# TechPizzaDev/VorbisPizza

Hardware: AMD Instinct MI355X
Metric: decoded PCM Msamples/s (batched stereo N=2048) (higher is better)
Workload: dtype f32; 1 GPU; north_star: batched stereo 44.1 kHz N=2048 IMDCT + window + overlap-add to PCM through the fused kernel (Mdct.Reverse + OverlapBuffers + StoreContiguous, Mdct.cs:15-19 + StreamDecoder.cs:764-791, 594-638): 65536 all-long frames x 2 ch per GPU (BASELINE configs[1]'s batch taken all the way to PCM), spectra N(0, 2^-8) device-resident, planar float32 PCM out, 8 B per sample; frames_per_gpu=65536, channels=2, block_size=2048, device_state=steady: 200 untimed steps of the workload in front of the W warm-up steps

## Files before the change

vorbispizza_amd/_build.py:

```python
import os
import subprocess
import sys

_HERE = os.path.dirname(os.path.abspath(__file__))
CSRC = os.path.join(_HERE, "csrc")
LIB_DIR = os.path.join(_HERE, "lib")
LIB_PATH = os.path.join(LIB_DIR, "libvorbispizza_synth.so")
OBJ_DIR = os.path.join(LIB_DIR, "obj")

SOURCES = {
    "imdct_fast.hip": [],
    "imdct_exact.hip": ["-ffp-contract=off"],
    "synth_kernels.hip": [],
    "synth_dual.hip": [],
    "synth_pairs.hip": [],
    "synth_big.hip": [],
    "floor0.hip": ["-ffp-contract=off"],
    "vpz_context.hip": ["-ffp-contract=off"],
    "vpz_decoder.hip": ["-ffp-contract=off"],
    "synth_plan.hip": ["-ffp-contract=off"],
    "entropy.hip": ["-ffp-contract=off"],
    "pcm_pack.hip": [],
    "pcm_resample.hip": [],
    "pcm_logmel.hip": [],
    "pcm_fbank.hip": [],
    "pcm_loudness.hip": [],
    "pcm_truepeak.hip": [],
    "pcm_featpost.hip": ["-ffp-contract=off"],
}
COMMON = ["--offload-arch=gfx950", "-O3", "-std=c++17", "-fPIC", "-Wall", "-Wno-unused-function",
          "-Wno-constant-logical-operand", "-fno-strict-aliasing"]


def _hipcc():
    for cand in (os.environ.get("HIPCC"), "/opt/rocm/bin/hipcc"):
        if cand and os.path.exists(cand):
            return cand
    return "hipcc"


def _deps(src):
    deps = [src]
    if os.path.basename(src) == "synth_pairs.hip":
        deps.append(os.path.join(CSRC, "synth_dual.hip"))
    for name in os.listdir(CSRC):
        if name.endswith(".hpp"):
            deps.append(os.path.join(CSRC, name))
    deps.append(os.path.join(_HERE, "..", "include", "vorbispizza_synth.h"))
# ... 90 lines not shown
```

vorbispizza_amd/csrc/imdct_core.hpp:

```cpp
#pragma once

#include <hip/hip_runtime.h>

namespace vpz {

constexpr float kSqrtHalf = 0.70710678118654752440f;

typedef float vpz_c2 __attribute__((ext_vector_type(2)));
__device__ __forceinline__ vpz_c2 c2(float2 a) { return vpz_c2{a.x, a.y}; }
__device__ __forceinline__ float2 f2(vpz_c2 a) { return make_float2(a.x, a.y); }
__device__ __forceinline__ vpz_c2 cadd_i(vpz_c2 a, vpz_c2 d)
{
    vpz_c2 r;
    asm("v_pk_add_f32 %0, %1, %2 op_sel:[0,1] op_sel_hi:[1,0] neg_lo:[0,1]" : "=v"(r) : "v"(a), "v"(d));
    return r;
}
__device__ __forceinline__ vpz_c2 csub_i(vpz_c2 a, vpz_c2 d)
{
    vpz_c2 r;
    asm("v_pk_add_f32 %0, %1, %2 op_sel:[0,1] op_sel_hi:[1,0] neg_hi:[0,1]" : "=v"(r) : "v"(a), "v"(d));
    return r;
}
__device__ __forceinline__ vpz_c2 cmul2(vpz_c2 a, vpz_c2 b)
{
// ... 106 lines not shown
    const int g = lane >> 3, l = lane & 7;
    float2 z[8];
    float2 tw[8];
#pragma unroll
    for (int m = 0; m < 8; ++m) tw[m] = s_tw[l + 8 * m];
#pragma unroll
    for (int m = 0; m < 8; ++m) {
        float re = lane_mirror8(xa[7 - m].y, lane);
        z[m] = cmul(make_float2(re, xa[m].x), tw[m]);
    }
    radix8_inverse(z);
#pragma unroll
    for (int p = 1; p < 8; ++p) z[p] = cmul(z[p], s_twBC[l * 8 + p]);
#pragma unroll
    for (int p = 0; p < 8; ++p) scratch[72 * g + 9 * p + l] = z[p];
#pragma unroll
    for (int r = 0; r < 8; ++r) z[r] = scratch[72 * g + 9 * l + r];
    radix8_inverse(z);
    float wim[8];
#pragma unroll
    for (int q = 0; q < 8; ++q) {
        float2 w = cmul(z[q], tw[q]);
        z[q].x = w.x;
        wim[q] = -w.y;
    }
    float *h = reinterpret_cast<float *>(scratch);
#pragma unroll
    for (int q = 0; q < 8; ++q) {
        float hi = lane_mirror8(wim[7 - q], lane);
        reinterpret_cast<float2 *>(h)[g * 64 + l + 8 * q] = make_float2(z[q].x, hi);
    }
}

__device__ __forceinline__ void imdct2048_wave_x2_regs(const float2 (&xa)[8], const float2 (&xb)[8], float2 *scratch_a, float2 *scratch_b,
                                                       const float2 (&tw)[8], const float2 (&twAB)[8], const float2 (&twBC)[8], int lane)
{
    float2 za[8], zb[8];
#pragma unroll
    for (int m = 0; m < 8; ++m) {
        const float ra = lane_mirror64(xa[7 - m].y, lane), rb = lane_mirror64(xb[7 - m].y, lane);
        za[m] = cmul(make_float2(ra, xa[m].x), tw[m]);
        zb[m] = cmul(make_float2(rb, xb[m].x), tw[m]);
    }
    {
        float2 *sa = scratch_a, *sb = scratch_b;
        radix8_inverse(za);
        radix8_inverse(zb);
#pragma unroll
        for (int p = 1; p < 8; ++p) {
            za[p] = cmul(za[p], twAB[p]);
            zb[p] = cmul(zb[p], twAB[p]);
        }
        const int l0 = lane & 7, pp = lane >> 3;
#pragma unroll
        for (int p = 0; p < 8; ++p) {
            sa[72 * p + lane] = za[p];
            sb[72 * p + lane] = zb[p];
        }
#pragma unroll
        for (int l1 = 0; l1 < 8; ++l1) {
            za[l1] = sa[72 * pp + l0 + 8 * l1];
            zb[l1] = sb[72 * pp + l0 + 8 * l1];
        }
        radix8_inverse(za);
        radix8_inverse(zb);
#pragma unroll
        for (int q = 1; q < 8; ++q) {
            za[q] = cmul(za[q], twBC[q]);
            zb[q] = cmul(zb[q], twBC[q]);
        }
#pragma unroll
        for (int q = 0; q < 8; ++q) {
            sa[66 * l0 + pp + 8 * q] = za[q];
            sb[66 * l0 + pp + 8 * q] = zb[q];
        }
#pragma unroll
        for (int r = 0; r < 8; ++r) {
            za[r] = sa[66 * r + lane];
            zb[r] = sb[66 * r + lane];
        }
        radix8_inverse(za);
        radix8_inverse(zb);
    }
    float wa[8], wb[8];
#pragma unroll
    for (int q = 0; q < 8; ++q) {
        const float2 a = cmul(za[q], tw[q]), b = cmul(zb[q], tw[q]);
        za[q].x = a.x;
        wa[q] = -a.y;
        zb[q].x = b.x;
        wb[q] = -b.y;
    }
#pragma unroll
    for (int q = 0; q < 8; ++q) {
        const float ha = lane_mirror64(wa[7 - q], lane), hb = lane_mirror64(wb[7 - q], lane);
        scratch_a[lane + 64 * q] = make_float2(za[q].x, ha);
        scratch_b[lane + 64 * q] = make_float2(zb[q].x, hb);
    }
}

__device__ __forceinline__ void imdct256_wave8_x2(const float2 (&xa)[8], const float2 (&xb)[8], float2 *scratch_a,
                                                  float2 *scratch_b, const float2 *s_tw, const float2 *s_twBC, int lane)
{
    const int g = lane >> 3, l = lane & 7;
    float2 za[8], zb[8];
    float2 tw[8];
#pragma unroll
    for (int m = 0; m < 8; ++m) tw[m] = s_tw[l + 8 * m];
#pragma unroll
    for (int m = 0; m < 8; ++m) {
        const float ra = lane_mirror8(xa[7 - m].y, lane), rb = lane_mirror8(xb[7 - m].y, lane);
        za[m] = cmul(make_float2(ra, xa[m].x), tw[m]);
        zb[m] = cmul(make_float2(rb, xb[m].x), tw[m]);
    }
    radix8_inverse(za);
    radix8_inverse(zb);
#pragma unroll
    for (int p = 1; p < 8; ++p) {
        const float2 w = s_twBC[l * 8 + p];
        za[p] = cmul(za[p], w);
        zb[p] = cmul(zb[p], w);
    }
#pragma unroll
    for (int p = 0; p < 8; ++p) {
        scratch_a[72 * g + 9 * p + l] = za[p];
        scratch_b[72 * g + 9 * p + l] = zb[p];
    }
#pragma unroll
    for (int r = 0; r < 8; ++r) {
        za[r] = scratch_a[72 * g + 9 * l + r];
// ... 176 lines not shown
```

vorbispizza_amd/csrc/synth_plan.hip:

```cpp
#include <cstdio>
#include <cstdlib>
#include <cstring>

#include "synth_plan.hpp"

namespace vpz {

constexpr int kCutSkewPermille = 25;

namespace {

constexpr int64_t kNone = INT64_MAX;


struct Prev {
    bool has_prev, prev_long;
    int prev_end, prev_stop;
};
inline Prev prev_of_state(const StreamState &S) { return Prev{S.has_prev, S.prev_long, S.prev_end, S.prev_stop}; }
inline Prev prev_of(const Decoder &D, const vpz_packet *packets, int64_t p)
{
    if (p > 0 && packets[p - 1].stream == packets[p].stream) {
        const vpz_packet &pp = packets[p - 1];
        const PacketInfo &ppi = D.packet_info[pp.flags & 7];
// ... 757 lines not shown
        }
        return n;
    };
    const bool want_inline = P.cut_R > 0 && P.cut_R + 1 <= 16;
    P.run_inline = want_inline ? arena_alloc<uint8_t>(*P.A, 32 * n_runs + 32) : nullptr;
    auto inline_range = [&](size_t lo, size_t hi) {
        for (size_t i = lo; want_inline && i < hi; ++i) {
            const RunDesc &r = runs[i];
            uint8_t *dst = P.run_inline + 32 * i;
            memset(dst, 0, 32);
            if (!(r.flags & kRunCompact)) continue;
            const int64_t q = (int64_t)r.first + (r.pre_kind == kPreRecompute ? -1 : 0);
            const int n = std::min(16, r.count + (r.pre_kind == kPreRecompute ? 1 : 0));
            for (int j = 0; j < n; ++j) {
                dst[j] = P.cflags[q + j];
                dst[16 + j] = P.cmap[q + j];
            }
        }
    };
    P.chain_threads = 1;
    if (P.pool && P.pool->parties() > 1 && n_runs >= 1024) {
        const int n_threads = P.chain_threads = P.pool->parties();
        std::vector<int64_t> part((size_t)n_threads, 0);
        P.host_failed |= !P.pool->run([&](int party) {
            const size_t lo = n_runs * (size_t)party / n_threads, hi = n_runs * (size_t)(party + 1) / n_threads;
            part[(size_t)party] = chain_range(lo, hi);
            inline_range(lo, hi);
        });
        for (int64_t v : part) P.n_chained += v;
    } else {
        P.n_chained = chain_range(0, n_runs);
        inline_range(0, n_runs);
    }
}

}

bool SynthPlan::dual_usable() const
{
    if (!D.dual_ok || (facts.any_floor0 && !D.f0_fused) || (facts.ilv_seen && facts.planar_seen)) return false;
    const bool wide = facts.ilv_seen && !D.pairs;
    const bool dev_ok = mem_space == VPZ_MEM_HOST || D.residue_format == VPZ_RESIDUE_I16 || (residue_addr & (wide ? 15 : 7)) == 0;
    if (!(dev_ok && (wide ? facts.group_align_ok : facts.align2_ok))) return false;
    if (D.pairs && !D.pairs_always && (facts.ilv_seen || out_interleaved)) return false;
    return true;
}
bool SynthPlan::group_usable() const
{
    return D.group_ok && facts.group_align_ok &&
           (mem_space == VPZ_MEM_HOST || D.residue_format == VPZ_RESIDUE_I16 || (residue_addr & 15) == 0);
}

int plan_frames(SynthPlan &P, int64_t *samples_written)
{
    int rc = run_state_machine_parallel(P, samples_written);
    if (rc < 0) return rc;
    P.was_parallel = rc == 1;
    if (rc == 0 && (rc = run_state_machine(P, samples_written)) != VPZ_OK) return rc;
    const bool wants_group = P.facts.need_coupling || (P.out_interleaved && P.D.channels > 2);
    P.use_dual = P.dual_usable();
    P.use_group = !P.use_dual && P.D.group_ok && wants_group && !P.facts.any_floor0 && P.facts.group_align_ok &&
                  (P.mem_space == VPZ_MEM_HOST || (P.residue_addr & 15) == 0);
    return VPZ_OK;
}

void plan_runs(SynthPlan &P)
// ... 4 lines not shown
    Cut c;
    cut_segments(P, c);
    P.cut_by_cost = c.batches;
    const int n_segs = (int)W.cut_segs.size();
    const size_t runs_arena_mark = P.A->used;
    for (int attempt = 0; attempt < 2; ++attempt) {
        P.A->used = runs_arena_mark;
        P.n_runs = 0;
        c.reuse = c.batches && c.parties > 1 && W.cut_hint_frames == total_frames && W.cut_hint_streams == D.n_streams &&
                  W.cut_hint_R > 0;
        if (c.batches && W.cut_code.size() < (size_t)total_frames) W.cut_code.resize((size_t)total_frames);
        if (c.batches) W.s_units.assign((size_t)n_segs, 0);
        c.total_units = (c.batches && !c.reuse) ? count_units(P, c) : 8 * total_frames;
        c.R = W.cut_hint_R;
        c.run_slots = W.cut_hint_slots;
        c.single_round = false;
        if (!c.reuse) choose_run_length(P, c);
        c.min_run_frames = std::max(1, c.R - 1 - (c.R >= 16 ? c.R * kCutSkewPermille / 1000 + 2 : 0));
        P.runs_cap = (size_t)(total_frames / c.min_run_frames) + (size_t)std::max(n_segs, D.n_streams) + 1;
        P.runs = arena_alloc<RunDesc>(*P.A, P.runs_cap);
        if (D.generic) return;
        fit_target(P, c);
        if (!c.batches && !c.skew_frames && P.pool && P.pool->parties() > 1 && total_frames / std::max(1, c.R) >= 1024)
            write_runs_by_length_wide(P, c);
        else
            write_runs_per_segment(P, c);
        if (P.host_failed) { P.n_runs = 0; return; }
        if (!(c.reuse && ((int64_t)P.n_runs > c.run_slots || (int64_t)P.n_runs * 10 < W.cut_hint_runs * 9))) break;
        W.cut_hint_frames = -1;
    }
    if (c.batches && !c.reuse) W.cut_hint_runs = (int64_t)P.n_runs;
    P.cut_R = c.R;
    chain_runs(P);
    if (getenv("VPZ_HOST_PROFILE"))
        fprintf(stderr, "[vpz host] cut: %s, by %s, R %d, target %lld eighths, %zu runs for %lld slots, %d segments on %d threads, heavy below %lld, "
                        "hint (frames %lld, runs %lld), chained %lld, runs filled by %s on %d threads, chain sweep on %d threads\n",
                c.reuse ? "hint reused" : "fitted", c.batches ? "cost" : "length", c.R,
                (long long)c.target_units, P.n_runs, (long long)c.run_slots, n_segs, c.parties, (long long)c.heavy_work,
                (long long)W.cut_hint_frames, (long long)W.cut_hint_runs, (long long)P.n_chained,
                P.fill_threads > 1 ? "the pool" : "the calling thread", P.fill_threads, P.chain_threads);
}

}
```

vorbispizza_amd/csrc/synth_plan.hpp:

```cpp
#pragma once

#include <algorithm>

#include "host_pool.hpp"
#include "vpz_decoder.hpp"

namespace vpz {

struct BatchFacts {
    bool any_floor = false, any_floor0 = false, need_coupling = false;
    bool any_short = false;
    bool ilv_seen = false, planar_seen = false;
    bool group_align_ok = true;
    bool align2_ok = true;
    int64_t res_extent = 0;
    void note(const Decoder &D, const vpz_packet &pk)
    {
        const bool bf = pk.flags & VPZ_PKT_BLOCK_FLAG;
        if (!bf) any_short = true;
        res_extent = std::max(res_extent, pk.residue_offset + (int64_t)D.channels * ((bf ? D.size1 : D.size0) / 2));
        if (!(pk.flags & VPZ_PKT_NO_FLOOR)) {
            any_floor = true;
            if (D.mappings[pk.mapping].coupling_steps > 0) need_coupling = true;
            if (D.mapping_uses_floor0[pk.mapping]) any_floor0 = true;
        }
        if (pk.flags & VPZ_PKT_INTERLEAVED) { need_coupling = true; ilv_seen = true; }
        else planar_seen = true;
        if (pk.residue_offset & 3) group_align_ok = false;
        if (pk.residue_offset & 1) align2_ok = false;
    }
    void merge(const BatchFacts &o)
    {
        any_floor |= o.any_floor; any_floor0 |= o.any_floor0; need_coupling |= o.need_coupling; any_short |= o.any_short;
        ilv_seen |= o.ilv_seen; planar_seen |= o.planar_seen; group_align_ok &= o.group_align_ok; align2_ok &= o.align2_ok;
        res_extent = std::max(res_extent, o.res_extent);
    }
};

struct SynthPlan {
    Decoder &D;
    const int64_t n_packets;
    const vpz_packet *packets;
    const bool have_posts;
    const int mem_space;
    const uintptr_t residue_addr;
    const bool out_interleaved;
    const int64_t stream_out_capacity;
    PinnedArena *A = nullptr;
    HostPool *pool = nullptr;
    int parties = 1;
    int dual_waves = 1;
    bool needs_general = false;
    int64_t (*resident_slots)(const SynthPlan &) = nullptr;
    std::vector<StreamState> st;
    std::vector<uint8_t> started_with_prev, started_prev_long;
    FrameDesc *frames = nullptr;
    size_t n_frames = 0;
    uint8_t *rec_floor = nullptr;
    BatchFacts facts;
    bool was_parallel = false;
    bool use_group = false;
    bool use_dual = false;
    bool cut_by_cost = false;
    bool compact = false;
    uint8_t *cflags = nullptr, *cmap = nullptr;
    uint8_t *run_inline = nullptr;
    RunDesc *runs = nullptr;
    size_t n_runs = 0, runs_cap = 0;
    bool host_failed = false;
    int64_t n_chained = 0;
    int cut_R = 0;
    int fill_threads = 1, chain_threads = 1;

    int64_t capacity_of(int s) const
    {
        return D.stream_caps.empty() ? stream_out_capacity : std::min(stream_out_capacity, D.stream_caps[(size_t)s]);
    }
    bool dual_usable() const;
    bool group_usable() const;
};

int plan_frames(SynthPlan &P, int64_t *samples_written);
void plan_runs(SynthPlan &P);

}
```

vorbispizza_amd/csrc/vpz_decoder.hip:

```cpp
#include <algorithm>
#include <chrono>
#include <cstdio>
#include <cstdlib>
#include <cstring>
#include <new>
#include <vector>

#include "synth_plan.hpp"
#include "../../include/vorbispizza_synth_debug.h"

namespace vpz {

static const uint32_t k_inverse_db_bits[256] = {
#include "floor1_inverse_db_bits.inc"
};

constexpr size_t kZeroCopyMax = 8u << 20;
__global__ __launch_bounds__(256) void widen_i16_kernel(const int16_t *__restrict__ in, float *__restrict__ out, long n)
{
    const long stride = (long)gridDim.x * 256 * 8;
    if ((reinterpret_cast<uintptr_t>(in) & 15) == 0) {
        for (long i = ((long)blockIdx.x * 256 + threadIdx.x) * 8; i < n; i += stride) {
            if (i + 8 <= n) {
                const uint4 v = *reinterpret_cast<const uint4 *>(in + i);
// ... 129 lines not shown
    if (cfg->floor_count < 0 || cfg->mapping_count < 0 || (cfg->floor_count && !cfg->floors && !cfg->floor_types) ||
        (cfg->mapping_count && !cfg->mappings) || cfg->mapping_count > 256 || cfg->floor_count > 64)
        return set_error(ctx, VPZ_E_INVALID_ARG, "vpz_decoder_create: bad floor / mapping tables");
    VPZ_HIP_TRY(ctx, hipSetDevice(ctx->device));

    vpz_decoder *d = new (std::nothrow) vpz_decoder();
    if (!d) return VPZ_E_NOMEM;
    Decoder &D = d->impl;
    D.ctx = ctx;
    D.channels = cfg->channels;
    D.size0 = cfg->block_size0;
    D.size1 = cfg->block_size1;
    D.clip = cfg->clip_samples ? 1 : 0;
    D.n_streams = n_streams;
    {
        const char *no_big = getenv("VPZ_NO_BIG");
        D.big = synth_big_supported(cfg->block_size0, cfg->block_size1) && !(no_big && atoi(no_big));
    }
    D.generic = !synth_supports_sizes(cfg->block_size0, cfg->block_size1) && !D.big;
    D.states.assign(n_streams, StreamState());
    D.floors.assign((size_t)cfg->floor_count, vpz_floor1_config{});
    D.floor_types.assign((size_t)cfg->floor_count, 1);
    D.floors0.assign((size_t)cfg->floor_count, vpz_floor0_config{});
    for (int i = 0; i < cfg->floor_count; ++i) {
        if (cfg->floor_types) D.floor_types[i] = cfg->floor_types[i];
        if (D.floor_types[i] == 1 && cfg->floors) D.floors[i] = cfg->floors[i];
        if (D.floor_types[i] == 0 && cfg->floors0) D.floors0[i] = cfg->floors0[i];
    }
    D.mappings.assign(cfg->mappings, cfg->mappings + cfg->mapping_count);
    static_assert(VPZ_PKT_BLOCK_FLAG == 1 && VPZ_PKT_PREV_FLAG == 2 && VPZ_PKT_NEXT_FLAG == 4, "packet_info index");
    for (int f = 0; f < 8; ++f) D.packet_info[f] = get_packet_info(D.size0, D.size1, f & 1, f & 2, f & 4);
    if (const char *e = getenv("VPZ_NO_DIRECT_I16")) D.no_direct_i16 = atoi(e) != 0;
    if (const char *e = getenv("VPZ_NO_CHAIN")) D.no_chain = atoi(e) != 0;
    if (const char *e = getenv("VPZ_DUAL_RUN")) D.dual_run = std::max(4, atoi(e));
    if (const char *e = getenv("VPZ_PLAN_SLOTS")) D.plan_slots = std::max<int64_t>(0, atoll(e));
    if (const char *e = getenv("VPZ_SYNTH_ABLATE")) D.ablate = atoi(e);
    if (const char *e = getenv("VPZ_HOST_THREADS")) D.host_threads = atoi(e);
    if (const char *e = getenv("VPZ_NO_EARLY_UPLOAD")) D.no_early_upload = atoi(e) != 0;
    if (const char *e = getenv("VPZ_PAR_MIN_PACKETS")) D.par_min_packets = atoll(e);

    int rc = VPZ_OK;
    std::vector<FloorDev> fdev(std::max<size_t>(1, D.floors.size()));
    for (size_t i = 0; i < D.floors.size() && rc == VPZ_OK; ++i) {
        if (D.floor_types[i] == 1) {
            rc = build_floor(D.floors[i], &fdev[i]);
        } else if (D.floor_types[i] == 0) {
            const vpz_floor0_config &f0 = D.floors0[i];
            if (f0.order < 1 || f0.order > 255 || f0.rate < 1 || f0.bark_map_size < 1 || f0.amp_bits < 0 || f0.amp_bits > 63)
                rc = VPZ_E_INVALID_ARG;
        } else {
            rc = VPZ_E_INVALID_ARG;
        }
    }
    std::vector<uint8_t> steps;
    for (size_t m = 0; m < D.mappings.size() && rc == VPZ_OK; ++m) {
        const vpz_mapping_config &mc = D.mappings[m];
        if (mc.coupling_steps < 0 || mc.coupling_steps > VPZ_MAX_COUPLING) { rc = VPZ_E_INVALID_ARG; break; }
        while (mc.coupling_steps && steps.size() % (2 * kStepsPadPairs)) steps.push_back(0);
        D.mapping_steps_off.push_back(mc.coupling_steps ? (int32_t)steps.size() : -1);
        for (int i = 0; i < mc.coupling_steps; ++i) {
            const int mag = mc.coupling_magnitude[i], ang = mc.coupling_angle[i];
            if (mag == ang || mag >= D.channels || ang >= D.channels) { rc = VPZ_E_INVALID_ARG; break; }
            steps.push_back((uint8_t)mag);
            steps.push_back((uint8_t)ang);
        }
        for (int ch = 0; ch < D.channels && rc == VPZ_OK; ++ch)
// ... 327 lines not shown
    GenericFrame *gf = nullptr;
    int64_t *src0 = nullptr, *dst0 = nullptr, *src1 = nullptr, *dst1 = nullptr;
    int32_t *save_list = nullptr;
    size_t n0 = 0, n1 = 0, n_save = 0;
    int64_t y_floats = 0;
    const float *d_res = nullptr, *d_amp = nullptr, *d_coeff = nullptr;
    const int16_t *d_posts = nullptr;
    const uint8_t *d_counts = nullptr;
    void *d_out = nullptr;
    bool early_residue = false, early_posts = false;
    bool spec_i16 = false;
    int64_t early_res_extent = 0;

    SynthCall(Decoder &dec, int64_t n, const vpz_packet *pk, const float *res, const int16_t *po, const uint8_t *pc,
              int mem, void *out, const int64_t *out_off, int64_t out_cap, int layout, int64_t stride)
        : D(dec), ctx(dec.ctx), n_packets(n), packets(pk), residue(res), posts(po), post_counts(pc), mem_space(mem),
          pcm_out(out), stream_out_offset(out_off), stream_out_capacity(out_cap), out_layout(layout),
          channel_stride(stride), C(dec.channels), half0(dec.size0 / 2), half1(dec.size1 / 2),
          n_rec(n * dec.channels), have_posts(po && pc && !dec.floors.empty()),
          out_interleaved(layout == VPZ_OUT_INTERLEAVED || layout == VPZ_OUT_INTERLEAVED_S16),
          out_s16(layout == VPZ_OUT_INTERLEAVED_S16 || layout == VPZ_OUT_PLANAR_S16),
          out_elem(out_s16 ? sizeof(int16_t) : sizeof(float)),
          P{dec, n, pk, have_posts, mem, reinterpret_cast<uintptr_t>(res), out_interleaved, out_cap}
    {
    }

    void *dev(const void *host_ptr) const
    {
        if (!host_ptr) return nullptr;
        char *base = zero_copy ? A->mapped : static_cast<char *>(A->dev.p);
        return base + (static_cast<const char *>(host_ptr) - A->base);
    }
    bool zero_copy = false;

    int resolved_parties = 0;
    int host_parties()
    {
        if (resolved_parties > 0) return resolved_parties;
        int parties = D.host_threads;
        if (parties <= 0) {
            cpu_set_t set;
            parties = sched_getaffinity(0, sizeof set, &set) == 0 ? CPU_COUNT(&set) : (int)std::thread::hardware_concurrency();
            if (const char *lw = getenv("LOCAL_WORLD_SIZE")) parties /= std::max(1, atoi(lw));
            parties = std::max(1, std::min(parties, 16));
        }
        return resolved_parties = parties;
    }
    HostPool *own_pool()
    {
        const int parties = host_parties();
        HostPool *pool = static_cast<HostPool *>(ctx->host_pool);
        if (n_packets >= D.par_min_packets && parties >= 2 && !(pool && pool->parties() == parties)) {
            if (pool) ctx->host_pool_free(pool);
            ctx->host_pool = pool = new HostPool(parties);
            ctx->host_pool_free = [](void *p) { delete static_cast<HostPool *>(p); };
        }
        return pool && parties >= 2 && pool->parties() == parties ? pool : nullptr;
    }

    int plan_frames(int64_t *samples_written)
    {
        P.A = A;
        P.pool = own_pool();
        P.parties = host_parties();
        P.dual_waves = synth_dual_waves();
        P.needs_general = synth_needs_general(D.size0, D.size1);
// ... 382 lines not shown
        a.f0_stride = D.f0_k;
        a.spec_i16 = spec_i16 ? 1 : 0;
        a.state_h = D.d_state_h;
        if (D.big && !P.use_dual) {
            const int64_t tf = synth_big_tail_floats(D.size1, (int64_t)P.n_runs * C);
            if (tf > 0) {
                const int grc = grow(ctx, D.b_bigtail, sizeof(float) * (size_t)tf);
                if (grc != VPZ_OK) return grc;
            }
            a.big_tail = static_cast<float *>(D.b_bigtail.p);
        }
        a.state_slot_floats = (int64_t)D.n_streams * C * half1;
        a.tw_long = D.t1->d_fast;
        a.tw_short = D.t0->d_fast;
        a.slope0 = D.t0->d_slope;
        a.slope1 = D.t1->d_slope;
        a.out = static_cast<float *>(d_out);
        a.stream_out_off = d_outoff;
        a.channel_stride = dev_channel_stride;
        a.interleaved = out_interleaved;
        a.s16 = out_s16 ? 1 : 0;
        a.clip = D.clip;
        a.clipped = D.d_clipped;
        a.no_batch = ((D.ablate & 128) || !P.cut_by_cost || P.facts.any_floor0) ? 1 : 0;
        a.ablate = D.ablate;
        a.stamps = nullptr;
#if defined(VPZ_STAMPS) || defined(VPZ_WAVE_TIMES)
        static unsigned long long *d_stamps = nullptr;
        constexpr size_t kStampWaves = 1 << 16;
        if (!d_stamps) (void)hipMalloc(&d_stamps, (16 + 16 * kStampWaves) * sizeof(unsigned long long));
        (void)hipMemsetAsync(d_stamps, 0, (16 + 16 * std::min<size_t>(kStampWaves, P.n_runs)) * sizeof(unsigned long long), ctx->stream);
        a.stamps = d_stamps;
#endif
        hipError_t e = P.use_dual ? (D.pairs ? launch_synth_pairs(a, P.facts.any_floor, P.facts.ilv_seen, ctx->stream) : launch_synth_dual(a, P.facts.any_floor, P.facts.ilv_seen, ctx->stream))
                                : D.big ? launch_synth_big(a, P.facts.any_floor, ctx->stream) : launch_synth(a, P.facts.any_floor, ctx->stream);
        if (e != hipSuccess) return set_error(ctx, VPZ_E_HIP, "synth kernel launch", e);
#if defined(VPZ_STAMPS) || defined(VPZ_WAVE_TIMES)
        {
            unsigned long long h[16];
            (void)hipMemcpyAsync(h, d_stamps, sizeof(h), hipMemcpyDeviceToHost, ctx->stream);
            (void)hipStreamSynchronize(ctx->stream);
            static const char *names_one[9] = {"desc+prefetch", "barrier0", "stage+barrier", "coupling", "pickup+curve",
                                               "floor*+imdct", "wait next", "ola+stores", "tail"};
            static const char *names_dual[9] = {"desc+prefetch", "unpack+coupling", "curves", "floor*+imdct x2", "wait next",
                                                "ola+stores", "tail", "-", "-"};
            const char **names = P.use_dual ? names_dual : names_one;
            unsigned long long tot = 0;
            for (int k = 0; k < 9; ++k) tot += h[k];
            fprintf(stderr, "[stamps] %llu waves, %.0f cycles per wave:", h[15], h[15] ? (double)tot / h[15] : 0.0);
            for (int k = 0; k < 9; ++k) fprintf(stderr, " %s %.1f%%", names[k], tot ? 100.0 * h[k] / tot : 0.0);
            if (h[14] && h[15]) {
                const double mean = (double)tot / h[15], var = (double)h[13] * 1e6 / h[15] - mean * mean;
                fprintf(stderr, " | slowest wave %.0f cycles = %.2f x mean, sigma %.2f x mean, %.1f passes per wave, %d runs", (double)h[14],
                        (double)h[14] / mean, var > 0 ? sqrt(var) / mean : 0.0, (double)h[12] / h[15], (int)P.n_runs);
            }
            fprintf(stderr, "\n");
            if (const char *dump = getenv("VPZ_STAMPS_DUMP")) {
                const size_t nw = std::min<size_t>(kStampWaves, P.n_runs);
                std::vector<unsigned long long> w(16 * nw);
                (void)hipMemcpy(w.data(), d_stamps + 16, w.size() * sizeof(unsigned long long), hipMemcpyDeviceToHost);
                if (FILE *f = fopen(dump, "w")) {
                    fprintf(f, "run,stream,frames,passes,long_frames,c0,c1,c2,c3,c4,c5,c6\n");
                    for (size_t r = 0; r < nw; ++r) {
                        fprintf(f, "%zu,%d,%d,%llu,%llu", r, P.runs[r].stream, P.runs[r].count, w[16 * r + 9], w[16 * r + 10]);
                        for (int k = 0; k < 7; ++k) fprintf(f, ",%llu", w[16 * r + k]);
                        fprintf(f, "\n");
                    }
// ... 78 lines not shown
    const auto t_arena = tick();
    if ((rc = call.plan_frames(samples_written)) != VPZ_OK) return rc;
    const SynthPlan &plan = call.P;
    if (plan.facts.res_extent > residue_floats)
        return set_error(ctx, VPZ_E_INVALID_ARG, "vpz_decoder_synth: a packet's residue lies beyond residue_floats");
    const auto t_pass1 = tick();
    if (plan.n_frames == 0) {
        D.states = plan.st;
        return VPZ_OK;
    }
    plan_runs(call.P);
    if (plan.host_failed) return set_error(ctx, VPZ_E_NOMEM, "vpz_decoder_synth: run cutting failed (allocation)");
    call.build_coupling_packets();
    if ((rc = call.build_floor0_records()) != VPZ_OK) return rc;
    if ((rc = call.build_output_offsets()) != VPZ_OK) return rc;
    call.build_generic_lists();
    const auto t_pass2 = tick();
    if ((rc = call.stage_inputs()) != VPZ_OK) return rc;
    if ((rc = call.launch()) != VPZ_OK) return rc;
    if (call.zero_copy) {
        VPZ_HIP_TRY(ctx, hipEventRecord(call.A->uploaded, ctx->stream));
        call.A->pending = true;
    }
    if ((rc = call.copy_back()) != VPZ_OK) return rc;
    early_guard.completed = mem_space == VPZ_MEM_HOST;
    if (!D.generic)
        for (int s = 0; s < D.n_streams; ++s)
            if (D.plan.s_cnt[s] > 0) call.P.st[s].state_slot ^= 1;
    D.states = plan.st;
    if (host_profile) {
        const auto t_end = tick();
        auto us = [](auto a, auto b) { return std::chrono::duration<double, std::micro>(b - a).count(); };
        const char *route = D.generic ? "generic" : plan.use_dual ? (D.pairs ? "pairs" : "stereo") : D.big ? "big" : plan.use_group ? "group" : "separate";
        fprintf(stderr, "[vpz host] packets %lld: route %s, arena wait %.1f us, pass1 %.1f us (%s), runs %.1f us, uploads+launch %.1f us\n",
                (long long)n_packets, route, us(t_begin, t_arena), us(t_arena, t_pass1), plan.was_parallel ? "parallel" : "serial",
                us(t_pass1, t_pass2), us(t_pass2, t_end));
    }
    return VPZ_OK;
}

int vpz_decoder_synth(vpz_decoder *d, int64_t n_packets, const vpz_packet *packets, const float *residue,
                      int64_t residue_floats, const int16_t *posts, const uint8_t *post_counts, int64_t n_records,
                      int mem_space, void *pcm_out, const int64_t *stream_out_offset, int64_t stream_out_capacity,
                      int out_layout, int64_t channel_stride, int64_t *samples_written)
{
    if (!d) return VPZ_E_INVALID_ARG;
    try {
        return synth_impl(d, n_packets, packets, residue, residue_floats, posts, post_counts, n_records, mem_space, pcm_out,
                          stream_out_offset, stream_out_capacity, out_layout, channel_stride, samples_written);
    } catch (const ArenaOverflow &) {
        return set_error(d->impl.ctx, VPZ_E_NOMEM, "vpz_decoder_synth: the descriptor arena is too small for this batch");
    } catch (const std::bad_alloc &) {
        return set_error(d->impl.ctx, VPZ_E_NOMEM, "vpz_decoder_synth: host allocation failed");
    } catch (...) {
        return set_error(d->impl.ctx, VPZ_E_NOMEM, "vpz_decoder_synth: host pass failed");
    }
}

int vpz_decoder_last_packet_status(vpz_decoder *d, int32_t *out, int64_t capacity, int64_t *n_not_ok)
{
    if (!d || capacity < 0 || (capacity > 0 && !out)) return VPZ_E_INVALID_ARG;
    Decoder &D = d->impl;
    const int64_t n = std::min<int64_t>(capacity, (int64_t)D.packet_samples.size());
    for (int64_t i = 0; i < n; ++i) out[i] = VPZ_OK;
    for (int64_t p : D.mismatch_packets)
        if (p < n) out[p] = VPZ_E_WINDOW_MISMATCH;
    if (n_not_ok) *n_not_ok = (int64_t)D.mismatch_packets.size();
    return VPZ_OK;
// ... 152 lines not shown
```

vorbispizza_amd/csrc/vpz_decoder.hpp:

```cpp
#pragma once

#include <vector>

#include "vpz_internal.hpp"

namespace vpz {

struct StreamState {
    bool has_prev = false;
    bool prev_long = false;
    int prev_start = 0, prev_end = 0, prev_stop = 0;
    int64_t current_position = 0;
    bool has_position = true;
    bool eos_found = false;
    bool has_clipped = false;
    int32_t clip_epoch = 1;
    int32_t state_slot = 0;
};

using DevBuf = Scratch;

struct PinnedArena {
    char *base = nullptr;
    char *mapped = nullptr;
// ... 63 lines not shown
    bool pairs_always = false;
    uint8_t *d_pair_ch = nullptr;
    uint32_t *d_pair_map_bits = nullptr;
    uint8_t *d_pair_steps = nullptr;
    int n_pair_step_pairs = 0;
    int max_steps = 0, n_step_pairs = 0;
    int host_threads = 0;
    int64_t par_min_packets = 16384;
    DevBuf b_in_res, b_in_posts, b_in_counts, b_out;
    DevBuf b_in_res16;
    int residue_format = VPZ_RESIDUE_F32;
    DevBuf b_ybuf;
    DevBuf b_bigtail;
    bool generic = false;
    bool big = false;
    std::vector<uint8_t> floor_types;
    std::vector<vpz_floor0_config> floors0;
    void *d_floors0 = nullptr;
    int32_t *d_bark_maps = nullptr;
    bool f0_fused = false;
    bool has_floor1 = false;
    int f0_k = 0;
    uint16_t *d_f0_bark = nullptr;
    float *d_f0_w = nullptr;
    DevBuf b_f0curve;
    DevBuf b_in_amp, b_in_coeff;
    const float *f0_amp = nullptr, *f0_coeff = nullptr;
    int32_t f0_stride = 0;
    PacketInfo packet_info[8];
    int dual_run = 8;
    int64_t plan_slots = 0;
    bool no_direct_i16 = false;
    bool no_chain = false;
    int ablate = 0;
    bool no_early_upload = false;
    std::vector<int32_t> packet_samples;
    std::vector<int64_t> mismatch_packets;
};

}
```

vorbispizza_amd/csrc/vpz_internal.hpp:

```cpp
#pragma once

#include <hip/hip_runtime.h>

#include <array>
#include <cstdint>
#include <map>
#include <string>
#include <utility>
#include <vector>

#include "../../include/vorbispizza_synth.h"
#include "../../include/vorbispizza_pcm_pack.h"
#include "synth_desc.hpp"

namespace vpz {

struct BlockTables {
    int n = 0;
    float2 *d_fast = nullptr;
    float *d_A = nullptr, *d_B = nullptr, *d_C = nullptr;
    uint16_t *d_bitrev = nullptr;
    int ld = 0;
    float *d_slope = nullptr;
    std::vector<float> h_slope;
// ... 91 lines not shown
                                 const int64_t *src_off = nullptr, const int64_t *dst_off = nullptr);
hipError_t launch_imdct_fast_4096(const float *spectra, float *out, int64_t count, const float2 *tw, Context *ctx,
                                  hipStream_t stream, const int64_t *src_off = nullptr, const int64_t *dst_off = nullptr);
hipError_t launch_imdct_fast_8192(const float *spectra, float *out, int64_t count, const float2 *tw, Context *ctx,
                                  hipStream_t stream, const int64_t *src_off = nullptr, const int64_t *dst_off = nullptr);
hipError_t launch_imdct_fast_mid(int n, const float *spectra, float *out, int64_t count, const float2 *tw, Context *ctx,
                                 hipStream_t stream, const int64_t *src_off = nullptr,
                                 const int64_t *dst_off = nullptr);
hipError_t launch_imdct_exact(int n, int ld, const float *spectra, float *out, int64_t count,
                              const float *A, const float *B, const float *C,
                              const uint16_t *bitrev, int num_cu, hipStream_t stream,
                              const int64_t *src_off = nullptr, const int64_t *dst_off = nullptr);

hipError_t launch_floor1_unwrap(int n_rec, const int16_t *posts, const uint8_t *post_counts, const uint8_t *rec_info,
                                const FloorDev *floors, int n_floors, int32_t *cposts, uint8_t *ccount, int16_t *dbg_y,
                                uint8_t *dbg_f, hipStream_t stream, int f0_fused = 0);
hipError_t launch_floor0_curves(int n_rec, const uint8_t *rec_info, const void *floors, const float *amp, const float *coeff,
                                int coeff_stride, int k_stride, const float *wtab, float *curve, const uint8_t *post_counts,
                                uint8_t *ccount, int32_t *cposts, hipStream_t stream);
hipError_t launch_floor0_wtab(const void *floors, int n_floors, int k_stride, float *wtab, hipStream_t stream);
hipError_t launch_floor1_render(int n_rec, const int32_t *cposts, const uint8_t *ccount, const uint8_t *rec_info,
                                int half0, int half1, uint8_t *curve_y, hipStream_t stream);
hipError_t launch_coupling(const void *pkts, int n_pkts, const uint8_t *steps, int channels,
                           const float *residue, float *temp, int max_half, hipStream_t stream);
hipError_t launch_synth(const SynthArgs &args, bool has_floor, hipStream_t stream);
bool synth_supports_sizes(int size0, int size1);
bool synth_needs_general(int size0, int size1);
int synth_resident_waves(bool has_floor, int num_cu, int channels, bool group);
bool synth_group_supported(int channels);
bool synth_dual_supported(int channels, int size0, int size1);
hipError_t launch_synth_dual(const SynthArgs &args, bool has_floor, bool interleaved_in, hipStream_t stream);
int synth_dual_resident_slots(bool has_floor, int num_cu);
int synth_dual_waves();
bool synth_pairs_supported(int channels, int size0, int size1);
hipError_t launch_synth_pairs(const SynthArgs &args, bool has_floor, bool interleaved_in, hipStream_t stream);
bool synth_big_supported(int size0, int size1);
hipError_t launch_synth_big(const SynthArgs &args, bool has_floor, hipStream_t stream);
int synth_big_resident_waves(bool has_floor, int num_cu, int size0, int size1);
int64_t synth_big_tail_floats(int size1, int64_t n_items);
hipError_t launch_generic_floor(const GenericFrame *frames, int n_frames, int channels, int half1, float *spec,
                                const uint8_t *post_counts, const uint8_t *curve_y, const float *inv_db,
                                hipStream_t stream);
hipError_t launch_generic_ola(const GenericFrame *frames, int n_frames, int channels, int size0, int size1,
                              const float *ybuf, float *state_y, const float *slope0, const float *slope1, float *out,
                              const int64_t *stream_out_off, int64_t channel_stride, int interleaved, int clip,
                              int32_t *clipped, int s16, hipStream_t stream);
hipError_t launch_generic_save_state(const GenericFrame *frames, const int32_t *save_list, int n_save, int channels,
                                     int size1, const float *ybuf, float *state_y, hipStream_t stream);
hipError_t launch_floor0_apply(const void *recs, int n_recs, const void *floors, const int32_t *bark_maps,
                               const float *amp, const float *coeff, int coeff_stride, float *spec,
                               hipStream_t stream);
size_t floor0_dev_size();
size_t floor0_rec_size();
void fill_floor0_dev(void *dst, int order, int bark_map_size, int amp_ofs, int64_t off_short, int64_t off_long);
void fill_floor0_rec(void *dst, int64_t spec_off, int rec, int floor, int half, int is_long);
size_t coupling_packet_size();
void fill_coupling_packet(void *dst, int64_t src_off, int64_t dst_off, int32_t half, int32_t steps_off,
                          int32_t steps, int32_t interleaved);

constexpr int kFastTwOffset = 0;
constexpr int kFastTwABOffset = 512;
constexpr int kFastTwBCOffset = 1024;
constexpr int kFastTableCount = 1024 + 64;
constexpr int kFast4096TwOffset = 0, kFast4096TwABOffset = 1024, kFast4096TwBCOffset = 1536, kFast4096WOffset = 1600;
constexpr int kFast4096TableCount = 2112;
constexpr int kFast8192TwOffset = 0, kFast8192TwABOffset = 2048, kFast8192TwBCOffset = 2560, kFast8192W1Offset = 2624,
// ... 9 lines not shown
```

Measured before the change: 609,000 Msamples/s.

## Add specialized steady-state stereo long-block synthesis kernel with register-resident overlap-add

Adds a dedicated kernel for the all-long, floorless, planar stereo 2048 case. It keeps previous-frame tails in registers, applies the window and overlap-add directly from the IMDCT outputs via lane mirroring, and writes PCM with nontemporal paired stores, skipping the scratch round-trip of the general dual path. Cross-wave neighbour handoff goes through shared memory with a spin-wait. The host plan detects eligibility and routes to it, and a compile-time sweep verifies the index maps. This adds a specialized code path and spin synchronization that could stall if assumptions fail.

New measurement: 696,400 Msamples/s (median of 6 runs). 1.14x the previous value.

```diff
diff --git a/vorbispizza_amd/_build.py b/vorbispizza_amd/_build.py
--- a/vorbispizza_amd/_build.py
+++ b/vorbispizza_amd/_build.py
@@ -14,6 +14,7 @@
     "synth_kernels.hip": [],
     "synth_dual.hip": [],
     "synth_pairs.hip": [],
+    "steady_stereo.hip": [],
     "synth_big.hip": [],
     "floor0.hip": ["-ffp-contract=off"],
     "vpz_context.hip": ["-ffp-contract=off"],
diff --git a/vorbispizza_amd/csrc/imdct_core.hpp b/vorbispizza_amd/csrc/imdct_core.hpp
--- a/vorbispizza_amd/csrc/imdct_core.hpp
+++ b/vorbispizza_amd/csrc/imdct_core.hpp
@@ -162,8 +162,9 @@
     }
 }
 
-__device__ __forceinline__ void imdct2048_wave_x2_regs(const float2 (&xa)[8], const float2 (&xb)[8], float2 *scratch_a, float2 *scratch_b,
-                                                       const float2 (&tw)[8], const float2 (&twAB)[8], const float2 (&twBC)[8], int lane)
+__device__ __forceinline__ void imdct2048_wave_x2_spectrum(const float2 (&xa)[8], const float2 (&xb)[8], float2 *scratch_a, float2 *scratch_b,
+                                                           const float2 (&tw)[8], const float2 (&twAB)[8], const float2 (&twBC)[8], int lane,
+                                                           float (&re_a)[8], float (&nim_a)[8], float (&re_b)[8], float (&nim_b)[8])
 {
     float2 za[8], zb[8];
 #pragma unroll
@@ -212,20 +213,26 @@
         radix8_inverse(za);
         radix8_inverse(zb);
     }
-    float wa[8], wb[8];
 #pragma unroll
     for (int q = 0; q < 8; ++q) {
         const float2 a = cmul(za[q], tw[q]), b = cmul(zb[q], tw[q]);
-        za[q].x = a.x;
-        wa[q] = -a.y;
-        zb[q].x = b.x;
-        wb[q] = -b.y;
-    }
+        re_a[q] = a.x;
+        nim_a[q] = -a.y;
+        re_b[q] = b.x;
+        nim_b[q] = -b.y;
+    }
+}
+
+__device__ __forceinline__ void imdct2048_wave_x2_regs(const float2 (&xa)[8], const float2 (&xb)[8], float2 *scratch_a, float2 *scratch_b,
+                                                       const float2 (&tw)[8], const float2 (&twAB)[8], const float2 (&twBC)[8], int lane)
+{
+    float ra[8], wa[8], rb[8], wb[8];
+    imdct2048_wave_x2_spectrum(xa, xb, scratch_a, scratch_b, tw, twAB, twBC, lane, ra, wa, rb, wb);
 #pragma unroll
     for (int q = 0; q < 8; ++q) {
         const float ha = lane_mirror64(wa[7 - q], lane), hb = lane_mirror64(wb[7 - q], lane);
-        scratch_a[lane + 64 * q] = make_float2(za[q].x, ha);
-        scratch_b[lane + 64 * q] = make_float2(zb[q].x, hb);
+        scratch_a[lane + 64 * q] = make_float2(ra[q], ha);
+        scratch_b[lane + 64 * q] = make_float2(rb[q], hb);
     }
 }
 
diff --git a/vorbispizza_amd/csrc/steady_map.hpp b/vorbispizza_amd/csrc/steady_map.hpp
--- /dev/null
+++ b/vorbispizza_amd/csrc/steady_map.hpp
@@ -0,0 +1,45 @@
+#pragma once
+
+namespace vpz {
+namespace steady {
+
+constexpr int kLanes = 64, kRegs = 8;
+constexpr int point(int lane, int q) { return lane + 64 * q; }
+constexpr int tail_index(int lane, int q) { return q < 4 ? 511 - 2 * point(lane, q) : 2 * point(lane, q) - 512; }
+constexpr int cur_index(int lane, int q) { return q < 4 ? 2 * point(lane, q) : 1023 - 2 * point(lane, q); }
+constexpr int sample_lo(int k) { return 511 - k; }
+constexpr int sample_hi(int k) { return 512 + k; }
+constexpr int kept_sample(int lane, int q) { return q < 4 ? sample_hi(cur_index(lane, q)) : sample_lo(cur_index(lane, q)); }
+constexpr int sent_sample(int lane, int q) { return q < 4 ? sample_lo(cur_index(lane, q)) : sample_hi(cur_index(lane, q)); }
+constexpr int store_index(int lane, int q) { return q < 4 ? 512 + 2 * point(lane, q) : 2 * point(lane, q) - 512; }
+
+constexpr bool sweep()
+{
+    bool tail_seen[512] = {}, sample_seen[1024] = {};
+    for (int q = 0; q < kRegs; ++q)
+        for (int l = 0; l < kLanes; ++l) {
+            const int t = tail_index(l, q), k = cur_index(l, q);
+            if (t < 0 || t >= 512 || tail_seen[t]) return false;
+            tail_seen[t] = true;
+            if (k < 0 || k >= 512) return false;
+            if (t != 511 - k) return false;
+            const int a = sample_lo(k), b = sample_hi(k);
+            if (a < 0 || a >= 512 || b < 512 || b >= 1024 || sample_seen[a] || sample_seen[b]) return false;
+            sample_seen[a] = sample_seen[b] = true;
+            const int pl = 63 - l, pq = 7 - q;
+            if (kept_sample(l, q) & 1) return false;
+            if (sent_sample(pl, pq) != kept_sample(l, q) + 1) return false;
+            if (store_index(l, q) != kept_sample(l, q)) return false;
+            const int j = point(l, q), ia = 2 * j, ib = 1023 - 2 * j;
+            if (q < 4 ? (ia != k || ib != 512 + t) : (ib != k || ia != 512 + t)) return false;
+        }
+    for (int i = 0; i < 512; ++i)
+        if (!tail_seen[i]) return false;
+    for (int i = 0; i < 1024; ++i)
+        if (!sample_seen[i]) return false;
+    return true;
+}
+static_assert(sweep(), "steady_stereo_kernel's index maps: tails a permutation of 0..511, samples of 0..1023, swap partners (63 - l, 7 - q)");
+
+}
+}
diff --git a/vorbispizza_amd/csrc/steady_stereo.hip b/vorbispizza_amd/csrc/steady_stereo.hip
--- /dev/null
+++ b/vorbispizza_amd/csrc/steady_stereo.hip
@@ -0,0 +1,223 @@
+#include "imdct_core.hpp"
+#include "steady_map.hpp"
+#include "synth_common.hpp"
+#include "synth_desc.hpp"
+#include "vpz_internal.hpp"
+
+namespace vpz {
+
+constexpr int kSteadyWaves = 4;
+constexpr int kSteadyThreads = 64 * kSteadyWaves;
+
+__global__ __launch_bounds__(kSteadyThreads, 2) void steady_stereo_kernel(SynthArgs a)
+{
+    __shared__ float2 s_scr[kSteadyWaves][2][kWaveScratchFloat2];
+    __shared__ int s_done[kSteadyWaves];
+
+    const int lane = threadIdx.x & 63;
+    const int wave = __builtin_amdgcn_readfirstlane(threadIdx.x >> 6);
+    const int run_idx = (int)blockIdx.x * kSteadyWaves + wave;
+    const bool active = run_idx < a.n_runs;
+    RunDesc run = a.runs[active ? run_idx : 0];
+    float2 rtw[8], rtwAB[8], rtwBC[8];
+    float w_lo[8], w_hi[8];
+    {
+        const VPZ_GLOBAL float2 *tw = (const VPZ_GLOBAL float2 *)a.tw_long;
+        const VPZ_GLOBAL float *sl = (const VPZ_GLOBAL float *)a.slope1;
+#pragma unroll
+        for (int m = 0; m < 8; ++m) {
+            rtw[m] = tw[kFastTwOffset + lane + 64 * m];
+            rtwAB[m] = tw[kFastTwABOffset + 64 * m + lane];
+            rtwBC[m] = tw[kFastTwBCOffset + 8 * (lane & 7) + m];
+            const int k = steady::cur_index(lane, m);
+            w_lo[m] = sl[steady::sample_lo(k)];
+            w_hi[m] = sl[steady::sample_hi(k)];
+        }
+    }
+    if (threadIdx.x < kSteadyWaves) s_done[threadIdx.x] = 0;
+    __syncthreads();
+    if (!active) return;
+
+    float2 *scrL = s_scr[wave][0], *scrR = s_scr[wave][1];
+    const int n_staged = run.count + (run.pre_kind == kPreRecompute ? 1 : 0);
+    const bool defer = run.pre_kind == kPreNeighbour && wave > 0 && run.count > 0;
+    const bool first_emits = run.pre_kind == kPreState;
+    const VPZ_GLOBAL float2 *src = (const VPZ_GLOBAL float2 *)(a.spec + run.spec_base);
+    const VPZ_GLOBAL float2 *idle = (const VPZ_GLOBAL float2 *)a.inv_db;
+    float *row_l, *row_r;
+    {
+        float *ob = a.out + (a.stream_out_off ? a.stream_out_off[run.stream] : 0) + run.out_base;
+        const uint64_t p = reinterpret_cast<uint64_t>(ob);
+        const uint32_t lo = __builtin_amdgcn_readfirstlane((uint32_t)p), hi = __builtin_amdgcn_readfirstlane((uint32_t)(p >> 32));
+        row_l = reinterpret_cast<float *>(((uint64_t)hi << 32) | lo);
+        row_r = row_l + a.channel_stride;
+    }
+    const bool clip_on = a.clip != 0;
+    float clip_peak = 0.0f;
+
+    float tL[8], tR[8];
+#pragma unroll
+    for (int q = 0; q < 8; ++q) tL[q] = tR[q] = 0.0f;
+    if (run.pre_kind == kPreState) {
+        const VPZ_GLOBAL float *st = (const VPZ_GLOBAL float *)(a.state_h + (size_t)run.state_slot * a.state_slot_floats + (size_t)run.stream * 2 * 1024);
+#pragma unroll
+        for (int q = 0; q < 8; ++q) {
+            tL[q] = st[steady::tail_index(lane, q)];
+            tR[q] = st[1024 + steady::tail_index(lane, q)];
+        }
+    }
+    float parkL[8], parkR[8];
+#pragma unroll
+    for (int q = 0; q < 8; ++q) parkL[q] = parkR[q] = 0.0f;
+
+    auto prefetch = [&](const VPZ_GLOBAL float2 *s2, bool valid, float2 (&va)[8], float2 (&vb)[8]) {
+        int l = lane;
+        asm volatile("" : "+v"(l));
+        const VPZ_GLOBAL float2 *p = valid ? s2 : idle;
+        const int base = valid ? l : 0, step = valid ? 64 : 0, rofs = valid ? 512 : 0;
+#pragma unroll
+        for (int m = 0; m < 8; ++m) {
+            va[m] = p[base + step * m];
+            vb[m] = p[base + step * m + rofs];
+        }
+    };
+    auto emit = [&](const float (&curL)[8], const float (&curR)[8], const float (&pL)[8], const float (&pR)[8], float *out_l, float *out_r) {
+        float loL[8], hiL[8], loR[8], hiR[8];
+#pragma unroll
+        for (int q = 0; q < 8; ++q) {
+            loL[q] = ola(-curL[q], w_lo[q], pL[q], w_hi[q]);
+            hiL[q] = ola(curL[q], w_hi[q], pL[q], w_lo[q]);
+            loR[q] = ola(-curR[q], w_lo[q], pR[q], w_hi[q]);
+            hiR[q] = ola(curR[q], w_hi[q], pR[q], w_lo[q]);
+        }
+        if (clip_on) {
+#pragma unroll
+            for (int q = 0; q < 8; q += 2) {
+                clip_group(loL[q], hiL[q], loL[q + 1], hiL[q + 1], clip_peak);
+                clip_group(loR[q], hiR[q], loR[q + 1], hiR[q + 1], clip_peak);
+            }
+        }
+        int lf = lane;
+        asm volatile("" : "+v"(lf));
+#pragma unroll
+        for (int q = 0; q < 8; ++q) {
+            const float gotL = lane_mirror64(q < 4 ? hiL[7 - q] : loL[7 - q], lf);
+            const float gotR = lane_mirror64(q < 4 ? hiR[7 - q] : loR[7 - q], lf);
+            const int at = q < 4 ? 512 + 2 * (lf + 64 * q) : 2 * (lf + 64 * q) - 512;
+            vpz_f2v vl = {q < 4 ? hiL[q] : loL[q], gotL}, vr = {q < 4 ? hiR[q] : loR[q], gotR};
+            __builtin_nontemporal_store(vl, (VPZ_GLOBAL vpz_f2v *)reinterpret_cast<vpz_f2v *>(out_l + at));
+            __builtin_nontemporal_store(vr, (VPZ_GLOBAL vpz_f2v *)reinterpret_cast<vpz_f2v *>(out_r + at));
+        }
+    };
+
+    float2 va[8], vb[8];
+    prefetch(src, n_staged > 0, va, vb);
+#pragma unroll
+    for (int m = 0; m < 8; ++m) asm volatile("" ::"v"(va[m].x), "v"(va[m].y), "v"(vb[m].x), "v"(vb[m].y));
+
+    float *out_l = row_l + (defer ? 1024 : 0), *out_r = row_r + (defer ? 1024 : 0);
+#ifdef VPZ_STAMPS
+    unsigned long long t_acc[12] = {0, 0, 0, 0, 0, 0, 0, 0, 0, 0, 0, 0};
+    unsigned long long t_last = __builtin_amdgcn_s_memtime();
+#endif
+    const int iters = n_staged;
+    for (int it = 0; it < iters; ++it) {
+        float2 na[8], nb[8];
+        src += 1024;
+        prefetch(src, it + 1 < iters, na, nb);
+        VPZ_STAMP(0);
+        int ln = lane;
+        asm volatile("" : "+v"(ln));
+        float reL[8], nimL[8], reR[8], nimR[8];
+        imdct2048_wave_x2_spectrum(va, vb, scrL, scrR, rtw, rtwAB, rtwBC, ln, reL, nimL, reR, nimR);
+        VPZ_STAMP(3);
+#pragma unroll
+        for (int m = 0; m < 8; ++m) asm volatile("" ::"v"(na[m].x), "v"(na[m].y), "v"(nb[m].x), "v"(nb[m].y));
+        VPZ_STAMP(4);
+        float curL[8], curR[8];
+#pragma unroll
+        for (int q = 0; q < 8; ++q) {
+            curL[q] = q < 4 ? reL[q] : nimL[q];
+            curR[q] = q < 4 ? reR[q] : nimR[q];
+        }
+        if (it > 0 || first_emits) {
+            emit(curL, curR, tL, tR, out_l, out_r);
+            out_l += 1024;
+            out_r += 1024;
+        } else if (defer) {
+#pragma unroll
+            for (int q = 0; q < 8; ++q) {
+                parkL[q] = curL[q];
+                parkR[q] = curR[q];
+            }
+        }
+        VPZ_STAMP(5);
+#pragma unroll
+        for (int q = 0; q < 8; ++q) {
+            tL[q] = q < 4 ? nimL[q] : reL[q];
+            tR[q] = q < 4 ? nimR[q] : reR[q];
+        }
+#pragma unroll
+        for (int m = 0; m < 8; ++m) {
+            va[m] = na[m];
+            vb[m] = nb[m];
+        }
+        VPZ_STAMP(6);
+    }
+#ifdef VPZ_STAMPS
+    if (a.stamps && lane == 0) {
+        unsigned long long tot = 0;
+        for (int k = 0; k < 9; ++k) { atomicAdd(&a.stamps[k], t_acc[k]); tot += t_acc[k]; }
+        atomicAdd(&a.stamps[15], 1ull);
+        atomicMax(&a.stamps[14], tot);
+        atomicAdd(&a.stamps[13], tot * tot / 1000000ull);
+        atomicAdd(&a.stamps[12], (unsigned long long)iters);
+    }
+#endif
+
+    {
+        float *pubL = reinterpret_cast<float *>(scrL), *pubR = reinterpret_cast<float *>(scrR);
+#pragma unroll
+        for (int q = 0; q < 8; ++q) {
+            pubL[64 * q + lane] = tL[q];
+            pubR[64 * q + lane] = tR[q];
+        }
+        __builtin_amdgcn_fence(__ATOMIC_RELEASE, "workgroup");
+        if (lane == 0) __hip_atomic_store(&s_done[wave], 1, __ATOMIC_RELAXED, __HIP_MEMORY_SCOPE_WORKGROUP);
+    }
+    if (defer) {
+        int spins = 0;
+        while (__hip_atomic_load(&s_done[wave - 1], __ATOMIC_RELAXED, __HIP_MEMORY_SCOPE_WORKGROUP) == 0 && ++spins < (1 << 23))
+            __builtin_amdgcn_s_sleep(4);
+        __builtin_amdgcn_fence(__ATOMIC_ACQUIRE, "workgroup");
+        const float *nbL = reinterpret_cast<const float *>(s_scr[wave - 1][0]), *nbR = reinterpret_cast<const float *>(s_scr[wave - 1][1]);
+        float pL[8], pR[8];
+#pragma unroll
+        for (int q = 0; q < 8; ++q) {
+            pL[q] = nbL[64 * q + lane];
+            pR[q] = nbR[64 * q + lane];
+        }
+        emit(parkL, parkR, pL, pR, row_l, row_r);
+    }
+    if (run.flags & kRunSaveState) {
+        VPZ_GLOBAL float *st = (VPZ_GLOBAL float *)(a.state_h + (size_t)(run.state_slot ^ 1) * a.state_slot_floats + (size_t)run.stream * 2 * 1024);
+#pragma unroll
+        for (int q = 0; q < 8; ++q) {
+            st[steady::tail_index(lane, q)] = tL[q];
+            st[1024 + steady::tail_index(lane, q)] = tR[q];
+        }
+    }
+    if (clip_on && __any(clip_peak > 0.99999994f) && lane == 0) atomicMax(&a.clipped[run.stream], run.clip_epoch);
+}
+
+hipError_t launch_steady_stereo(const SynthArgs &args, hipStream_t stream)
+{
+    if (args.n_runs <= 0) return hipSuccess;
+    if (args.channels != 2 || args.size0 != 256 || args.size1 != 2048 || args.interleaved || args.s16 || args.spec_i16 || args.ccount != nullptr)
+        return hipErrorInvalidValue;
+    const int grid = (args.n_runs + kSteadyWaves - 1) / kSteadyWaves;
+    hipLaunchKernelGGL(steady_stereo_kernel, dim3(grid), dim3(kSteadyThreads), 0, stream, args);
+    return hipGetLastError();
+}
+
+}
diff --git a/vorbispizza_amd/csrc/synth_plan.hip b/vorbispizza_amd/csrc/synth_plan.hip
--- a/vorbispizza_amd/csrc/synth_plan.hip
+++ b/vorbispizza_amd/csrc/synth_plan.hip
@@ -813,6 +813,20 @@
         P.n_chained = chain_range(0, n_runs);
         inline_range(0, n_runs);
     }
+}
+
+bool all_steady(const SynthPlan &P, const Cut &c)
+{
+    const Decoder &D = P.D;
+    if (!P.use_dual || D.pairs || !P.compact || c.batches || D.no_steady || D.channels != 2 || D.size0 != 256 || D.size1 != 2048) return false;
+    if (!P.facts.all_steady_flags || P.facts.any_floor || P.facts.any_short || P.facts.ilv_seen || !D.mismatch_packets.empty()) return false;
+    for (int s = 0; s < D.n_streams; ++s) {
+        if (D.plan.s_cnt[s] <= 0) continue;
+        const StreamState &S = D.states[s];
+        if (S.has_prev && !(S.prev_long && S.prev_end == 1024 && S.prev_stop == 2048)) return false;
+        if (D.plan.trim_out_count[s] >= 0) return false;
+    }
+    return true;
 }
 
 }
@@ -883,6 +897,7 @@
     if (c.batches && !c.reuse) W.cut_hint_runs = (int64_t)P.n_runs;
     P.cut_R = c.R;
     chain_runs(P);
+    P.steady = all_steady(P, c);
     if (getenv("VPZ_HOST_PROFILE"))
         fprintf(stderr, "[vpz host] cut: %s, by %s, R %d, target %lld eighths, %zu runs for %lld slots, %d segments on %d threads, heavy below %lld, "
                         "hint (frames %lld, runs %lld), chained %lld, runs filled by %s on %d threads, chain sweep on %d threads\n",
diff --git a/vorbispizza_amd/csrc/synth_plan.hpp b/vorbispizza_amd/csrc/synth_plan.hpp
--- a/vorbispizza_amd/csrc/synth_plan.hpp
+++ b/vorbispizza_amd/csrc/synth_plan.hpp
@@ -13,6 +13,7 @@
     bool ilv_seen = false, planar_seen = false;
     bool group_align_ok = true;
     bool align2_ok = true;
+    bool all_steady_flags = true;
     int64_t res_extent = 0;
     void note(const Decoder &D, const vpz_packet &pk)
     {
@@ -28,11 +29,13 @@
         else planar_seen = true;
         if (pk.residue_offset & 3) group_align_ok = false;
         if (pk.residue_offset & 1) align2_ok = false;
+        if ((pk.flags & (7u | VPZ_PKT_NO_FLOOR | VPZ_PKT_INTERLEAVED)) != (7u | VPZ_PKT_NO_FLOOR)) all_steady_flags = false;
     }
     void merge(const BatchFacts &o)
     {
         any_floor |= o.any_floor; any_floor0 |= o.any_floor0; need_coupling |= o.need_coupling; any_short |= o.any_short;
         ilv_seen |= o.ilv_seen; planar_seen |= o.planar_seen; group_align_ok &= o.group_align_ok; align2_ok &= o.align2_ok;
+        all_steady_flags &= o.all_steady_flags;
         res_extent = std::max(res_extent, o.res_extent);
     }
 };
@@ -69,6 +72,7 @@
     size_t n_runs = 0, runs_cap = 0;
     bool host_failed = false;
     int64_t n_chained = 0;
+    bool steady = false;
     int cut_R = 0;
     int fill_threads = 1, chain_threads = 1;
 
diff --git a/vorbispizza_amd/csrc/vpz_decoder.hip b/vorbispizza_amd/csrc/vpz_decoder.hip
--- a/vorbispizza_amd/csrc/vpz_decoder.hip
+++ b/vorbispizza_amd/csrc/vpz_decoder.hip
@@ -185,6 +185,7 @@
     for (int f = 0; f < 8; ++f) D.packet_info[f] = get_packet_info(D.size0, D.size1, f & 1, f & 2, f & 4);
     if (const char *e = getenv("VPZ_NO_DIRECT_I16")) D.no_direct_i16 = atoi(e) != 0;
     if (const char *e = getenv("VPZ_NO_CHAIN")) D.no_chain = atoi(e) != 0;
+    if (const char *e = getenv("VPZ_NO_STEADY")) D.no_steady = atoi(e) != 0;
     if (const char *e = getenv("VPZ_DUAL_RUN")) D.dual_run = std::max(4, atoi(e));
     if (const char *e = getenv("VPZ_PLAN_SLOTS")) D.plan_slots = std::max<int64_t>(0, atoll(e));
     if (const char *e = getenv("VPZ_SYNTH_ABLATE")) D.ablate = atoi(e);
@@ -578,6 +579,7 @@
         return base + (static_cast<const char *>(host_ptr) - A->base);
     }
     bool zero_copy = false;
+    bool steady_kernel = false;
 
     int resolved_parties = 0;
     int host_parties()
@@ -1026,7 +1028,16 @@
         (void)hipMemsetAsync(d_stamps, 0, (16 + 16 * std::min<size_t>(kStampWaves, P.n_runs)) * sizeof(unsigned long long), ctx->stream);
         a.stamps = d_stamps;
 #endif
-        hipError_t e = P.use_dual ? (D.pairs ? launch_synth_pairs(a, P.facts.any_floor, P.facts.ilv_seen, ctx->stream) : launch_synth_dual(a, P.facts.any_floor, P.facts.ilv_seen, ctx->stream))
+        steady_kernel = false;
+        if (P.steady && !out_interleaved && !out_s16 && !spec_i16) {
+            int64_t bits = (int64_t)reinterpret_cast<uintptr_t>(d_out) / (int64_t)sizeof(float) | dev_channel_stride;
+            if (reinterpret_cast<uintptr_t>(d_out) % sizeof(float)) bits |= 1;
+            for (int s = 0; s < D.n_streams; ++s)
+                if (D.plan.s_cnt[s] > 0) bits |= offs[s];
+            steady_kernel = (bits & 1) == 0;
+        }
+        hipError_t e = steady_kernel ? launch_steady_stereo(a, ctx->stream)
+                     : P.use_dual ? (D.pairs ? launch_synth_pairs(a, P.facts.any_floor, P.facts.ilv_seen, ctx->stream) : launch_synth_dual(a, P.facts.any_floor, P.facts.ilv_seen, ctx->stream))
                                 : D.big ? launch_synth_big(a, P.facts.any_floor, ctx->stream) : launch_synth(a, P.facts.any_floor, ctx->stream);
         if (e != hipSuccess) return set_error(ctx, VPZ_E_HIP, "synth kernel launch", e);
 #if defined(VPZ_STAMPS) || defined(VPZ_WAVE_TIMES)
@@ -1171,8 +1182,8 @@
         const auto t_end = tick();
         auto us = [](auto a, auto b) { return std::chrono::duration<double, std::micro>(b - a).count(); };
         const char *route = D.generic ? "generic" : plan.use_dual ? (D.pairs ? "pairs" : "stereo") : D.big ? "big" : plan.use_group ? "group" : "separate";
-        fprintf(stderr, "[vpz host] packets %lld: route %s, arena wait %.1f us, pass1 %.1f us (%s), runs %.1f us, uploads+launch %.1f us\n",
-                (long long)n_packets, route, us(t_begin, t_arena), us(t_arena, t_pass1), plan.was_parallel ? "parallel" : "serial",
+        fprintf(stderr, "[vpz host] packets %lld: route %s, kernel %s, arena wait %.1f us, pass1 %.1f us (%s), runs %.1f us, uploads+launch %.1f us\n",
+                (long long)n_packets, route, call.steady_kernel ? "steady" : "general", us(t_begin, t_arena), us(t_arena, t_pass1), plan.was_parallel ? "parallel" : "serial",
                 us(t_pass1, t_pass2), us(t_pass2, t_end));
     }
     return VPZ_OK;
diff --git a/vorbispizza_amd/csrc/vpz_decoder.hpp b/vorbispizza_amd/csrc/vpz_decoder.hpp
--- a/vorbispizza_amd/csrc/vpz_decoder.hpp
+++ b/vorbispizza_amd/csrc/vpz_decoder.hpp
@@ -119,6 +119,7 @@
     int64_t plan_slots = 0;
     bool no_direct_i16 = false;
     bool no_chain = false;
+    bool no_steady = false;
     int ablate = 0;
     bool no_early_upload = false;
     std::vector<int32_t> packet_samples;
diff --git a/vorbispizza_amd/csrc/vpz_internal.hpp b/vorbispizza_amd/csrc/vpz_internal.hpp
--- a/vorbispizza_amd/csrc/vpz_internal.hpp
+++ b/vorbispizza_amd/csrc/vpz_internal.hpp
@@ -147,6 +147,7 @@
 hipError_t launch_synth_dual(const SynthArgs &args, bool has_floor, bool interleaved_in, hipStream_t stream);
 int synth_dual_resident_slots(bool has_floor, int num_cu);
 int synth_dual_waves();
+hipError_t launch_steady_stereo(const SynthArgs &args, hipStream_t stream);
 bool synth_pairs_supported(int channels, int size0, int size1);
 hipError_t launch_synth_pairs(const SynthArgs &args, bool has_floor, bool interleaved_in, hipStream_t stream);
 bool synth_big_supported(int size0, int size1);
```
